# tianrluo/MRphy.py

Hardware: NVIDIA B200
Metric: spin_steps_per_sec_fwd_bwd (higher is better)
Workload: dtype f32

## Files before the change

mrphy.py_b200/csrc/blochsim_fused.cu:

```cuda
#include <cuda_runtime.h>
#include <stdint.h>
#include <stdio.h>
#include <stdlib.h>
#include <string.h>

#include "../../include/mrphy_b200.h"
#include "abi_common.cuh"
#define MRPHY_VOTE_MASK 0xffffffffu
#ifndef MRPHY_TC_MIN_NC
#define MRPHY_TC_MIN_NC 4
#endif
#include "bloch_math.cuh"
#include "ptx_helpers.cuh"
#include "tc_helpers.cuh"
#include "grad_finalize.cuh"

namespace mrphy {

#ifndef MRPHY_TCMAX1
#define MRPHY_TCMAX1 128
#endif
constexpr int TCMAX = 64;
template <typename T, int NC> struct ChunkMax { static constexpr int v = (sizeof(T) == 4 && NC == 1) ? MRPHY_TCMAX1 : TCMAX; };

#ifdef MRPHY_CTA_TRACE
__device__ unsigned long long g_cta_trace[8192][4];
__device__ __forceinline__ unsigned long long gtime() {
  unsigned long long t;
  asm volatile("mov.u64 %0, %globaltimer;" : "=l"(t));
  return t;
}
__device__ __forceinline__ unsigned smid() {
  unsigned s;
  asm volatile("mov.u32 %0, %smid;" : "=r"(s));
  return s;
}
#endif

template <typename T, int PK> struct Pack { typedef T type; };
template <> struct Pack<float, 2> { typedef f2 type; };

template <typename T, int W> struct WaveLayout {
  static constexpr bool STEPMAJOR = W * sizeof(T) > 44;
  static constexpr int WS = STEPMAJOR ? ((W + 3) & ~3) : W;
};
template <typename T, int W>
__device__ __forceinline__ void load_step(const T* wb, int TCP, int j, T (&sv)[W]) {
  if constexpr (WaveLayout<T, W>::STEPMAJOR) {
    constexpr int WS = WaveLayout<T, W>::WS;
    T tmp[WS];
    const float4* src = reinterpret_cast<const float4*>(wb + (size_t)j * WS);
    float4* dst = reinterpret_cast<float4*>(tmp);
#pragma unroll
    for (int e = 0; e < WS * (int)sizeof(T) / 16; ++e) dst[e] = src[e];
#pragma unroll
    for (int w = 0; w < W; ++w) sv[w] = tmp[w];
  } else {
#pragma unroll
    for (int w = 0; w < W; ++w) sv[w] = wb[w * TCP + j];
  }
}

#ifndef MRPHY_RED_BUDGET
#define MRPHY_RED_BUDGET 10240
#endif
#ifndef MRPHY_NC2_MINB
#define MRPHY_NC2_MINB 14
#endif
#ifndef MRPHY_WRED_TR_BYTES
#define MRPHY_WRED_TR_BYTES 64
#endif
#ifndef MRPHY_MC_MINB
#define MRPHY_MC_MINB 1
#endif
#ifndef MRPHY_BWD_MINB
#define MRPHY_BWD_MINB 8
#endif
#ifndef MRPHY_BWD_BLKT
#define MRPHY_BWD_BLKT 128
#endif
constexpr int pick_tr(int W, int elem) {
  int tr = 16;
  const int budget = W >= 19 ? 2 * MRPHY_RED_BUDGET : (W == 11 ? MRPHY_RED_BUDGET + 1024 : (W == 7 ? MRPHY_RED_BUDGET + 4096 : MRPHY_RED_BUDGET));
  while (tr > 1 && W * tr * 32 * elem > budget) tr >>= 1;
  return tr;
}

template <typename T, int NC, int BLKT, int PK = 1> struct BwdSmem {
  static constexpr int W = 2 * NC + 3;
  static constexpr int NW = BLKT / 32;
  static constexpr bool WRED = NC > 1 && PK == 1;
  static constexpr int TR = WRED ? MRPHY_WRED_TR_BYTES / (int)sizeof(T) : pick_tr(W, (int)sizeof(T));
  static constexpr int WP = (W + 3) & ~3;
  static constexpr int E16 = (int)sizeof(T) / 4;
  static constexpr int P16 = TR * E16 + 1;
  static constexpr size_t red_bytes = WRED ? (size_t)NW * 32 * (P16 * 16 + WP * sizeof(T)) : (size_t)NW * W * TR * 32 * sizeof(T);
  static constexpr size_t wbuf = 0;
  static constexpr int WS = WaveLayout<T, W>::WS;
  static constexpr int TCM = ChunkMax<T, NC>::v;
  static constexpr size_t red = (2 * WS * TCM * sizeof(T) + 127) / 128 * 128;
  static constexpr size_t cta = (red + red_bytes + 15) / 16 * 16;
  static constexpr size_t bar = (cta + (size_t)2 * NW * W * TR * sizeof(T) + 15) / 16 * 16;
  static constexpr size_t bytes = bar + 16;
};

template <typename T> struct KArgs {
  int N, nM, nT, K, TCP, nChunks, P;
  int chunk_elems;
  const T* Mi; int64_t Mi_sn, Mi_sm;
  const T* loc; int64_t loc_sn, loc_sm;
  const T* b1; int64_t b1_sn, b1_sm; int nC;
  mrphy_param df, T1, T2, gamma, dt;
  T* Mo;
  T* ckpt;
  const T* wave;
  const T* gMo; int64_t gMo_sn, gMo_sm;
  T* gMi;
  T* partials;
  int* sched;
  int n_sm, c_per_sm;
  int* done;
};
template <typename T> struct SgOut {
  T* gloc; T* gsz; T* gb1;
  bool any() const { return gloc || gsz || gb1; }
};
template <typename T> struct RecOut {
  T* Mt; const T* gMt;
  int every, nR;
};

constexpr int SCHED_SM_SLOTS = 256;
constexpr int SCHED_NCLAIMED = 256;
constexpr int SCHED_CLAIM = 264;
__device__ __forceinline__ unsigned my_smid() {
  unsigned s;
  asm volatile("mov.u32 %0, %%smid;" : "=r"(s));
  return s;
}

__device__ __forceinline__ void load4(const float* p, float (&v)[4]) {
  const float4 q = *reinterpret_cast<const float4*>(p);
  v[0] = q.x; v[1] = q.y; v[2] = q.z; v[3] = q.w;
}
__device__ __forceinline__ void load4(const double* p, double (&v)[4]) {
  const double2 a = *reinterpret_cast<const double2*>(p);
  const double2 b = *reinterpret_cast<const double2*>(p + 2);
  v[0] = a.x; v[1] = a.y; v[2] = b.x; v[3] = b.y;
}

template <int Q> __device__ __forceinline__ float getq(f2 a) { return Q == 0 ? a.v.x : a.v.y; }
template <int Q> __device__ __forceinline__ float getq(float a) { return a; }
template <int Q> __device__ __forceinline__ double getq(double a) { return a; }
__device__ __forceinline__ f2 mkv(float a, float b, f2*) { return f2(a, b); }
__device__ __forceinline__ float mkv(float a, float, float*) { return a; }
__device__ __forceinline__ double mkv(double a, double, double*) { return a; }

template <typename T, int NC, bool RELAX>
__device__ __forceinline__ void load_spin(const KArgs<T>& a, int n, int i, T lx, T ly, T lz, SpinConst<T, NC>& k) {
  T br[NC], bi[NC];
  if (a.b1) {
    const T* bp = a.b1 + (int64_t)n * a.b1_sn + (int64_t)i * a.b1_sm;
#pragma unroll
    for (int c = 0; c < NC; ++c) {
      br[c] = c < a.nC ? bp[c] : (T)0;
      bi[c] = c < a.nC ? bp[a.nC + c] : (T)0;
    }
  }
  const double gam = ld_param(a.gamma, n, i);
  const double dt = ld_param(a.dt, n, 0);
  const double df = a.df.ptr ? ld_param(a.df, n, i) : 0.0;
  const double t1 = RELAX ? ld_param(a.T1, n, i) : 1.0;
  const double t2 = RELAX ? ld_param(a.T2, n, i) : 1.0;
  make_consts<T, NC>(k, gam, dt, RELAX, t1, t2, df, lx, ly, lz, a.b1 ? br : nullptr, a.b1 ? bi : nullptr);
}
template <typename T, typename V, int NC, int PK, bool RELAX>
__device__ __forceinline__ void load_consts_v(const KArgs<T>& a, int n, const int (&idx)[PK], V lx, V ly, V lz,
                                              SpinConst<V, NC>& k) {
  if constexpr (PK == 1) {
    load_spin<T, NC, RELAX>(a, n, idx[0], lx, ly, lz, k);
  } else {
    SpinConst<float, NC> k0, k1;
    load_spin<float, NC, RELAX>(a, n, idx[0], getq<0>(lx), getq<0>(ly), getq<0>(lz), k0);
    load_spin<float, NC, RELAX>(a, n, idx[1], getq<1>(lx), getq<1>(ly), getq<1>(lz), k1);
    k = pack2<NC>(k0, k1);
  }
}
template <typename T, typename V, int PK>
__device__ __forceinline__ void load_vec3(const T* base, int64_t stride, const int (&idx)[PK], V& x, V& y, V& z) {
  const T* p0 = base + (int64_t)idx[0] * stride;
  const T* p1 = base + (int64_t)idx[PK - 1] * stride;
  x = mkv(p0[0], p1[0], (V*)nullptr);
  y = mkv(p0[1], p1[1], (V*)nullptr);
  z = mkv(p0[2], p1[2], (V*)nullptr);
}

template <typename T, typename V, int PK, int BLKT>
__device__ __forceinline__ void load_vec3_tile(const T* base, int64_t stride, int tile, int nM, const int (&idx)[PK],
                                               T* scr, V& x, V& y, V& z) {
  constexpr int TILE = BLKT * PK;
  const T* src = base + (int64_t)tile * TILE * 3;
  const bool coop = stride == 3 && (tile + 1) * TILE <= nM && (reinterpret_cast<uintptr_t>(src) & 15) == 0;
  if (coop) {
    constexpr int NVEC = TILE * 3 * (int)sizeof(T) / 16;
    const float4* s4 = reinterpret_cast<const float4*>(src);
    float4* d4 = reinterpret_cast<float4*>(scr);
    for (int q = threadIdx.x; q < NVEC; q += BLKT) d4[q] = s4[q];
    __syncthreads();
    const int l0 = threadIdx.x, l1 = (PK - 1) * BLKT + threadIdx.x;
    x = mkv(scr[3 * l0], scr[3 * l1], (V*)nullptr);
    y = mkv(scr[3 * l0 + 1], scr[3 * l1 + 1], (V*)nullptr);
    z = mkv(scr[3 * l0 + 2], scr[3 * l1 + 2], (V*)nullptr);
    __syncthreads();
  } else {
    load_vec3<T, V, PK>(base, stride, idx, x, y, z);
  }
}

template <typename T, typename V, int PK>
__device__ __forceinline__ void rec_store(const RecOut<T>& o, int nM, int n, int r, const int (&idx)[PK], const bool (&ok)[PK],
                                          V x, V y, V z) {
  T* p = o.Mt + ((size_t)n * o.nR + r) * 3 * (size_t)nM;
  if (ok[0]) {
    __stcs(p + idx[0], getq<0>(x));
    __stcs(p + (size_t)nM + idx[0], getq<0>(y));
    __stcs(p + 2 * (size_t)nM + idx[0], getq<0>(z));
  }
  if (PK == 2 && ok[PK - 1]) {
    __stcs(p + idx[PK - 1], getq<1>(x));
    __stcs(p + (size_t)nM + idx[PK - 1], getq<1>(y));
    __stcs(p + 2 * (size_t)nM + idx[PK - 1], getq<1>(z));
  }
}
template <typename T, typename V, int NC, int PK>
__device__ __forceinline__ void rec_load(const RecOut<T>& o, int nM, int n, int r, const int (&idx)[PK], const bool (&ok)[PK],
                                         const SpinConst<V, NC>& k, V& x, V& y, V& z) {
  const T* p = o.gMt + ((size_t)n * o.nR + r) * 3 * (size_t)nM;
  T v[PK][3];
#pragma unroll
  for (int q = 0; q < PK; ++q) {
#pragma unroll
    for (int e = 0; e < 3; ++e) v[q][e] = ok[q] ? __ldcs(p + e * (size_t)nM + idx[q]) : (T)0;
  }
  x = mkv(v[0][0], v[PK - 1][0], (V*)nullptr);
  y = mkv(v[0][1], v[PK - 1][1], (V*)nullptr);
  z = mkv(v[0][2], v[PK - 1][2], (V*)nullptr);
  to_frame(k, x, y);
}

template <typename T>
__global__ void pack_waveform_kernel(const T* __restrict__ rf, int64_t rf_sn, int64_t rf_sx, int64_t rf_st, int64_t rf_sc,
                                     const T* __restrict__ gr, int64_t gr_sn, int64_t gr_sx, int64_t gr_st, int nC,
                                     int NC, int sum_coils, int nT, int K, int TCP, int nChunks, int WS, int stepmajor,
                                     int64_t total, T* __restrict__ wave) {
  const int W = 2 * NC + 3;
  for (int64_t e = (int64_t)blockIdx.x * blockDim.x + threadIdx.x; e < total; e += (int64_t)gridDim.x * blockDim.x) {
    const int j = stepmajor ? (int)((e / WS) % TCP) : (int)(e % TCP);
    const int w = stepmajor ? (int)(e % WS) : (int)((e / TCP) % WS);
    const int c = (int)((e / ((int64_t)TCP * WS)) % nChunks);
    const int n = (int)(e / ((int64_t)TCP * WS * nChunks));
    const int t = c * K + j;
    T v = (T)0;
    if (j < K && t < nT && w < W) {
      if (w < 2 * NC) {
        const int x = w / NC, coil = w % NC;
        const T* p = rf + n * rf_sn + x * rf_sx + t * rf_st;
        if (sum_coils) {
          for (int q = 0; q < nC; ++q) v += p[q * rf_sc];
        } else if (coil < nC) {
          v = p[coil * rf_sc];
        }
      } else {
        v = gr[n * gr_sn + (w - 2 * NC) * gr_sx + t * gr_st];
      }
    }
    wave[e] = v;
  }
}

template <typename T, int POL, bool RELAX, int NC, int PK, int BLKT, bool REC = false>
__global__ void __launch_bounds__(BLKT, (PK == 2 ? (NC == 1 ? 14 : MRPHY_NC2_MINB) : 1)) fused_fwd_kernel(const KArgs<T> a, const RecOut<T> rec) {
  typedef typename Pack<T, PK>::type V;
  constexpr int W = 2 * NC + 3;
  constexpr int WS = WaveLayout<T, W>::WS;
  __shared__ __align__(128) T wbuf[2][WS * ChunkMax<T, NC>::v];
  __shared__ __align__(16) T scr[3 * BLKT * PK];
  __shared__ __align__(8) uint64_t full[2];
  const int tid = threadIdx.x, n = blockIdx.y;
  const int TCP = a.TCP, K = a.K, nT = a.nT, nChunks = a.nChunks, nM = a.nM;
  const uint32_t chunk_bytes = (uint32_t)(WS * TCP * sizeof(T));
  const T* wave_n = a.wave + (size_t)n * nChunks * WS * TCP;
  const int tiles = (nM + BLKT * PK - 1) / (BLKT * PK);
  const int my_tiles = ((int)blockIdx.x < tiles) ? (tiles - (int)blockIdx.x + (int)gridDim.x - 1) / (int)gridDim.x : 0;
  const uint32_t total = (uint32_t)my_tiles * (uint32_t)nChunks;
  if (tid == 0) {
    mbar_init(&full[0], 1);
    mbar_init(&full[1], 1);
    fence_barrier_init();
  }
  __syncthreads();
  if (tid == 0 && total > 0) {
    mbar_arrive_expect_tx(&full[0], chunk_bytes);
    bulk_g2s(wbuf[0], wave_n, chunk_bytes, &full[0]);
  }
  uint32_t it = 0;
  for (int tile = blockIdx.x; tile < tiles; tile += gridDim.x) {
    SpinConst<V, NC> k;
    V mx, my, mz;
    int idx[PK];
    bool ok[PK];
#pragma unroll
    for (int q = 0; q < PK; ++q) {
      const int i = (tile * PK + q) * BLKT + tid;
      ok[q] = i < nM;
      idx[q] = ok[q] ? i : nM - 1;
    }
    {
      V lx, ly, lz;
      load_vec3_tile<T, V, PK, BLKT>(a.loc + (int64_t)n * a.loc_sn, a.loc_sm, tile, nM, idx, scr, lx, ly, lz);
      load_consts_v<T, V, NC, PK, RELAX>(a, n, idx, lx, ly, lz, k);
    }
    load_vec3_tile<T, V, PK, BLKT>(a.Mi + (int64_t)n * a.Mi_sn, a.Mi_sm, tile, nM, idx, scr, mx, my, mz);
    to_frame(k, mx, my);
    int rc = rec.every, rr = 0;
    for (int c = 0; c < nChunks; ++c, ++it) {
      if (tid == 0 && it + 1 < total) {
        const int cn = (c + 1 == nChunks) ? 0 : c + 1;
        const uint32_t sn = (it + 1) & 1;
        mbar_arrive_expect_tx(&full[sn], chunk_bytes);
        bulk_g2s(wbuf[sn], wave_n + (size_t)cn * WS * TCP, chunk_bytes, &full[sn]);
      }
      mbar_wait(&full[it & 1], (it >> 1) & 1);
      const T* wb = wbuf[it & 1];
      const int ns = min(K, nT - c * K);
      auto one_step = [&](const T (&s)[W]) {
        V rx[NC], ry[NC], bx, by, bz;
#pragma unroll
        for (int q = 0; q < NC; ++q) { rx[q] = V(s[q]); ry[q] = V(s[NC + q]); }
        field<V, NC>(k, rx, ry, V(s[2 * NC]), V(s[2 * NC + 1]), V(s[2 * NC + 2]), bx, by, bz);
        step_fwd<V, POL, RELAX>(bx, by, bz, k.e1, k.e2, mx, my, mz);
        if constexpr (REC) {
          if (--rc == 0) {
            V x = mx, y = my;
            from_frame(k, x, y);
            rec_store<T, V, PK>(rec, nM, n, rr++, idx, ok, x, y, mz);
            rc = rec.every;
          }
        }
      };
      int j = 0;
      constexpr bool VEC4 = !WaveLayout<T, W>::STEPMAJOR;
      for (; VEC4 && j + 4 <= ns; j += 4) {
        T wv[W][4];
#pragma unroll
        for (int w = 0; w < W; ++w) load4(wb + w * TCP + j, wv[w]);
#pragma unroll
        for (int u = 0; u < 4; ++u) {
          T s[W];
#pragma unroll
          for (int w = 0; w < W; ++w) s[w] = wv[w][u];
          one_step(s);
        }
      }
      for (; j < ns; ++j) {
        T s[W];
        load_step<T, W>(wb, TCP, j, s);
        one_step(s);
      }
      if (c + 1 < nChunks) {
        T* cp = a.ckpt + ((size_t)n * (nChunks - 1) + c) * 3 * (size_t)nM;
        if (ok[0]) {
          __stcs(cp + idx[0], getq<0>(mx));
          __stcs(cp + (size_t)nM + idx[0], getq<0>(my));
          __stcs(cp + 2 * (size_t)nM + idx[0], getq<0>(mz));
        }
        if (PK == 2 && ok[PK - 1]) {
          __stcs(cp + idx[PK - 1], getq<1>(mx));
          __stcs(cp + (size_t)nM + idx[PK - 1], getq<1>(my));
          __stcs(cp + 2 * (size_t)nM + idx[PK - 1], getq<1>(mz));
        }
      }
      __syncthreads();
    }
    from_frame(k, mx, my);
    if (ok[0]) {
      T* op = a.Mo + ((size_t)n * nM + idx[0]) * 3;
      op[0] = getq<0>(mx); op[1] = getq<0>(my); op[2] = getq<0>(mz);
    }
    if (PK == 2 && ok[PK - 1]) {
      T* op = a.Mo + ((size_t)n * nM + idx[PK - 1]) * 3;
      op[0] = getq<1>(mx); op[1] = getq<1>(my); op[2] = getq<1>(mz);
    }
  }
}

template <typename T, int W, int TR, int W0 = 0, int W1 = W>
__device__ __forceinline__ void warp_tile_reduce(const T (*tile)[TR][32], int lane, T (*out)[TR]) {
  if constexpr (sizeof(T) == 4 && TR == 16) {
    const int r = lane >> 1, half = (lane & 1) << 4;
#pragma unroll
    for (int w = W0; w < W1; ++w) {
      const float4* row = reinterpret_cast<const float4*>(&tile[w][r][half]);
      T sum = (T)0;
#pragma unroll
      for (int q = 0; q < 4; ++q) {
        const float4 v = row[(q + r) & 3];
        sum += (v.x + v.y) + (v.z + v.w);
      }
      sum += __shfl_xor_sync(0xffffffffu, sum, 1);
      if (!(lane & 1)) out[w][r] = sum;
    }
  } else {
    const int r = lane & (TR - 1), grp = lane & ~(TR - 1);
#pragma unroll
    for (int w = W0; w < W1; ++w) {
      T sum = (T)0;
#pragma unroll
      for (int q = 0; q < TR; ++q) sum += tile[w][r][grp + ((q + lane) & (TR - 1))];
#pragma unroll
      for (int o = TR; o < 32; o <<= 1) sum += __shfl_xor_sync(0xffffffffu, sum, o);
      if (lane < TR) out[w][r] = sum;
    }
  }
}

template <typename T, int NC, int TR, int W0, int W1>
__device__ __forceinline__ void warp_tile_reduce_weighted(const unsigned char* ft, const T* wt, int lane, T (*out)[TR]) {
  constexpr int W = 2 * NC + 3, WP = (W + 3) & ~3, E16 = (int)sizeof(T) / 4, P16 = TR * E16 + 1, SP = TR;
  constexpr bool WANT_RF = W0 == 0, WANT_GR = W1 == W;
  const int r = lane % TR, grp = lane / TR;
  T acc[W];
#pragma unroll
  for (int w = 0; w < W; ++w) acc[w] = (T)0;
#pragma unroll 2
  for (int q = 0; q < SP; ++q) {
    const int sp = grp * SP + q;
    T f[4];
    {
      const float4* src = reinterpret_cast<const float4*>(ft + ((size_t)sp * P16 + (size_t)r * E16) * 16);
      float4* dst = reinterpret_cast<float4*>(f);
#pragma unroll
      for (int e = 0; e < E16; ++e) dst[e] = src[e];
    }
    T wv[WP];
    {
      const float4* src = reinterpret_cast<const float4*>(wt + (size_t)sp * WP);
      float4* dst = reinterpret_cast<float4*>(wv);
#pragma unroll
      for (int e = 0; e < WP * (int)sizeof(T) / 16; ++e) dst[e] = src[e];
    }
    if constexpr (WANT_RF) {
#pragma unroll
      for (int c = 0; c < NC; ++c) {
        acc[c] = fma_(wv[c], f[0], fma_(wv[NC + c], f[1], acc[c]));
        acc[NC + c] = fma_(wv[c], f[1], fnma_(wv[NC + c], f[0], acc[NC + c]));
      }
    }
    if constexpr (WANT_GR) {
      acc[2 * NC] = fma_(wv[2 * NC], f[2], acc[2 * NC]);
      acc[2 * NC + 1] = fma_(wv[2 * NC + 1], f[2], acc[2 * NC + 1]);
      acc[2 * NC + 2] = fma_(wv[2 * NC + 2], f[2], acc[2 * NC + 2]);
    }
  }
#pragma unroll
  for (int w = W0; w < W1; ++w) {
    T sum = acc[w];
#pragma unroll
    for (int o = TR; o < 32; o <<= 1) sum += __shfl_xor_sync(0xffffffffu, sum, o);
    if (lane < TR) out[w][r] = sum;
  }
}

template <typename T, typename V, int NC, int PK>
__device__ __forceinline__ void sg_fold(const KArgs<T>& a, const SgOut<T>& o, int n, const int (&idx)[PK], const bool (&ok)[PK], bool first,
                                        bool last, const SpinConst<V, NC>& k, const V (&acc)[4 + 2 * NC]) {
  constexpr int NA = 4 + 2 * NC;
#pragma unroll
  for (int q = 0; q < PK; ++q) {
    if (!ok[q]) continue;
    const size_t s = (size_t)n * a.nM + idx[q];
    T v[NA];
#pragma unroll
    for (int w = 0; w < NA; ++w) v[w] = q == 0 ? getq<0>(acc[w]) : getq<1>(acc[w]);
    T* const pl = o.gloc ? o.gloc + s * 3 : nullptr;
    T* const pz = o.gsz ? o.gsz + s : nullptr;
    T* const pb = o.gb1 ? o.gb1 + s * 2 * a.nC : nullptr;
    if (!first) {
      if (pl) { v[0] += pl[0]; v[1] += pl[1]; v[2] += pl[2]; }
      if (pz) v[3] += pz[0];
      if (pb) {
#pragma unroll
        for (int c = 0; c < NC; ++c)
          if (c < a.nC) { v[4 + c] += pb[c]; v[4 + NC + c] += pb[a.nC + c]; }
      }
    }
    if (last) {
      const T ng = (T)(-6.283185307179586476925286766559 * ld_param(a.gamma, n, idx[q]) * ld_param(a.dt, n, 0));
#pragma unroll
      for (int w = 0; w < NA; ++w) v[w] *= ng;
      if (NC == 1) {
        const T fc = q == 0 ? getq<0>(k.fc) : getq<1>(k.fc), fs = q == 0 ? getq<0>(k.fs) : getq<1>(k.fs);
        const T re = v[4], im = v[5];
        v[4] = fnma_(fs, im, fc * re);
        v[5] = fma_(fs, re, fc * im);
      }
    }
    if (pl) { pl[0] = v[0]; pl[1] = v[1]; pl[2] = v[2]; }
    if (pz) pz[0] = v[3];
    if (pb) {
#pragma unroll
      for (int c = 0; c < NC; ++c)
        if (c < a.nC) { pb[c] = v[4 + c]; pb[a.nC + c] = v[4 + NC + c]; }
    }
  }
}

template <typename T, int POL, bool RELAX, int NC, int PK, int BLKT, int ROWS = 3, bool SG = false, bool REC = false>
__global__ void __launch_bounds__(BLKT, (PK == 2 ? MRPHY_BWD_MINB * 64 / BLKT : (sizeof(T) == 8 && NC == 1 ? 4 : (sizeof(T) == 4 && NC > 1 ? MRPHY_MC_MINB : 1)))) fused_bwd_kernel(const KArgs<T> a, const int need_gmi, const SgOut<T> sgo, const RecOut<T> rec) {
  typedef typename Pack<T, PK>::type V;
  using L = BwdSmem<T, NC, BLKT, PK>;
  constexpr int W = L::W, TR = L::TR, NW = L::NW;
  constexpr bool WANT_RF = (ROWS & 1) != 0, WANT_GR = (ROWS & 2) != 0;
  constexpr int W0 = WANT_RF ? 0 : 2 * NC, W1 = WANT_GR ? W : 2 * NC;
  extern __shared__ __align__(128) unsigned char smem_raw[];
  constexpr int WS = L::WS;
  T(*wbuf)[WS * L::TCM] = reinterpret_cast<T(*)[WS * L::TCM]>(smem_raw + L::wbuf);
  T(*red)[W][TR][32] = reinterpret_cast<T(*)[W][TR][32]>(smem_raw + L::red);
  constexpr bool WRED = L::WRED;
  unsigned char* const ft = smem_raw + L::red + (size_t)(threadIdx.x >> 5) * 32 * L::P16 * 16;
  T* const wt = reinterpret_cast<T*>(smem_raw + L::red + (size_t)NW * 32 * L::P16 * 16) + (size_t)(threadIdx.x >> 5) * 32 * L::WP;
  T(*cta)[W][TR] = reinterpret_cast<T(*)[W][TR]>(smem_raw + L::cta);
  uint64_t* full = reinterpret_cast<uint64_t*>(smem_raw + L::bar);
  __shared__ __align__(16) T scr[3 * BLKT * PK];
  const int tid = threadIdx.x, lane = tid & 31, warp = tid >> 5, n = blockIdx.y;
  const int TCP = a.TCP, K = a.K, nT = a.nT, nChunks = a.nChunks, nM = a.nM;
  const uint32_t chunk_bytes = (uint32_t)(WS * TCP * sizeof(T));
  const T* wave_n = a.wave + (size_t)n * nChunks * WS * TCP;
  const int tiles = (nM + BLKT * PK - 1) / (BLKT * PK);
#define NCTA ((int)gridDim.x)
  __shared__ int s_vid, s_sweep;
  if (tid == 0) {
    mbar_init(&full[0], 1);
    mbar_init(&full[1], 1);
    fence_barrier_init();
  }
  if (a.done && blockIdx.x == 0 && tid == 0) a.done[n] = 0;
  int vid = blockIdx.x;
  if (a.sched && tid == 0) {
    int* const sched = a.sched;
    s_sweep = 0;
    const int s = (int)my_smid();
    int v0 = -1;
    if (s < a.n_sm && s < SCHED_SM_SLOTS) {
      const int rank = atomicAdd(&sched[s], 1);
      const int cand = rank * a.n_sm + s;
      if (rank < a.c_per_sm && cand < NCTA && atomicCAS(&sched[SCHED_CLAIM + cand], 0, 1) == 0) {
        v0 = cand;
        atomicAdd(&sched[SCHED_NCLAIMED], 1);
      }
    }
    s_vid = v0;
  }
  __syncthreads();
  if (a.sched) vid = s_vid;
#ifdef MRPHY_CTA_TRACE
  if (tid == 0 && blockIdx.x < 8192 && n == 0) { g_cta_trace[blockIdx.x][0] = smid(); g_cta_trace[blockIdx.x][1] = gtime(); g_cta_trace[blockIdx.x][3] = (unsigned long long)(long long)vid; }
#endif
  uint32_t it = 0, red_par = 0;
  for (;;) {
   if (vid >= 0) {
    const int my_tiles = (vid < tiles) ? (tiles - vid + NCTA - 1) / NCTA : 0;
    const uint32_t total = it + (uint32_t)my_tiles * (uint32_t)nChunks;
    T* part = a.partials + ((size_t)n * a.P + vid) * W * (size_t)nT;
    if (my_tiles == 0) {
      if constexpr (ROWS != 0)
        for (int e = tid; e < W * nT; e += BLKT) part[e] = (T)0;
    } else if (tid == 0) {
      mbar_arrive_expect_tx(&full[it & 1], chunk_bytes);
      bulk_g2s(wbuf[it & 1], wave_n + (size_t)(nChunks - 1) * WS * TCP, chunk_bytes, &full[it & 1]);
    }
  bool first = true;
  for (int tile = vid; tile < tiles; tile += NCTA, first = false) {
    SpinConst<V, NC> k;
    V mx, my, mz, hx, hy, hz;
    int idx[PK];
    bool ok[PK];
#pragma unroll
    for (int q = 0; q < PK; ++q) {
      const int i = (tile * PK + q) * BLKT + tid;
      ok[q] = i < nM;
      idx[q] = ok[q] ? i : nM - 1;
    }
    {
      V lx, ly, lz;
      load_vec3_tile<T, V, PK, BLKT>(a.loc + (int64_t)n * a.loc_sn, a.loc_sm, tile, nM, idx, scr, lx, ly, lz);
      load_consts_v<T, V, NC, PK, RELAX>(a, n, idx, lx, ly, lz, k);
    }
    load_vec3_tile<T, V, PK, BLKT>(a.Mo + (size_t)n * nM * 3, 3, tile, nM, idx, scr, mx, my, mz);
    load_vec3_tile<T, V, PK, BLKT>(a.gMo + (int64_t)n * a.gMo_sn, a.gMo_sm, tile, nM, idx, scr, hx, hy, hz);
    to_frame(k, mx, my);
    to_frame(k, hx, hy);
    if constexpr (WRED && ROWS != 0) {
      T* wrow = wt + (size_t)lane * L::WP;
#pragma unroll
      for (int q = 0; q < NC; ++q) { wrow[q] = lane0(k.cbr[q]); wrow[NC + q] = lane0(k.cbi[q]); }
      wrow[2 * NC] = lane0(k.glx); wrow[2 * NC + 1] = lane0(k.gly); wrow[2 * NC + 2] = lane0(k.glz);
#pragma unroll
      for (int q = W; q < L::WP; ++q) wrow[q] = (T)0;
      __syncwarp();
    }
    {
      const T z0 = ok[0] ? (T)1 : (T)0, z1 = ok[PK - 1] ? (T)1 : (T)0;
      const V zm = mkv(z0, z1, (V*)nullptr);
      hx = hx * zm; hy = hy * zm; hz = hz * zm;
    }
    int rc = 0, rr = 0;
    V gx, gy, gz;
    if constexpr (REC) {
      rc = nT - rec.nR * rec.every;
      rr = rec.nR - 1;
      rec_load<T, V, NC, PK>(rec, nM, n, rr, idx, ok, k, gx, gy, gz);
    }
    for (int c = nChunks - 1; c >= 0; --c, ++it) {
      if (tid == 0 && it + 1 < total) {
        const int cn = (c == 0) ? nChunks - 1 : c - 1;
        const uint32_t sn = (it + 1) & 1;
        mbar_arrive_expect_tx(&full[sn], chunk_bytes);
        bulk_g2s(wbuf[sn], wave_n + (size_t)cn * WS * TCP, chunk_bytes, &full[sn]);
      }
      V kx = mx, ky = my, kz = mz;
      if (c > 0) {
        const T* cp = a.ckpt + ((size_t)n * (nChunks - 1) + (c - 1)) * 3 * (size_t)nM;
        kx = mkv(__ldcs(cp + idx[0]), __ldcs(cp + idx[PK - 1]), (V*)nullptr);
        ky = mkv(__ldcs(cp + (size_t)nM + idx[0]), __ldcs(cp + (size_t)nM + idx[PK - 1]), (V*)nullptr);
        kz = mkv(__ldcs(cp + 2 * (size_t)nM + idx[0]), __ldcs(cp + 2 * (size_t)nM + idx[PK - 1]), (V*)nullptr);
      }
      mbar_wait(&full[it & 1], (it >> 1) & 1);
      const T* wb = wbuf[it & 1];
      const int ns = min(K, nT - c * K);
      V sacc[SG ? 4 + 2 * NC : 1];
      if constexpr (SG) {
#pragma unroll
        for (int w = 0; w < 4 + 2 * NC; ++w) sacc[w] = V(0.0f);
      }
      auto one_step = [&](const T (&s)[W], int row) {
        if constexpr (REC) {
          if (rc == 0) {
            hx = hx + gx; hy = hy + gy; hz = hz + gz;
            if (--rr >= 0) rec_load<T, V, NC, PK>(rec, nM, n, rr, idx, ok, k, gx, gy, gz);
            rc = rec.every;
          }
          --rc;
        }
        V rx[NC], ry[NC], bx, by, bz, Fx, Fy, Fz;
#pragma unroll
        for (int q = 0; q < NC; ++q) { rx[q] = V(s[q]); ry[q] = V(s[NC + q]); }
        field<V, NC>(k, rx, ry, V(s[2 * NC]), V(s[2 * NC + 1]), V(s[2 * NC + 2]), bx, by, bz);
        step_bwd<V, POL, RELAX, NC>(k, bx, by, bz, mx, my, mz, hx, hy, hz, Fx, Fy, Fz);
        if constexpr (SG) {
          sacc[0] = fma_(V(s[2 * NC]), Fz, sacc[0]);
          sacc[1] = fma_(V(s[2 * NC + 1]), Fz, sacc[1]);
          sacc[2] = fma_(V(s[2 * NC + 2]), Fz, sacc[2]);
          sacc[3] = sacc[3] + Fz;
#pragma unroll
          for (int q = 0; q < NC; ++q) {
            sacc[4 + q] = fma_(rx[q], Fx, fma_(ry[q], Fy, sacc[4 + q]));
            sacc[4 + NC + q] = fma_(rx[q], Fy, fnma_(ry[q], Fx, sacc[4 + NC + q]));
          }
        }
        if constexpr (ROWS == 0) return;
        if constexpr (WRED) {
          T fv[4] = {lane0(Fx), lane0(Fy), lane0(Fz), (T)0};
          float4* dst = reinterpret_cast<float4*>(ft + ((size_t)lane * L::P16 + (size_t)row * L::E16) * 16);
          const float4* src = reinterpret_cast<const float4*>(fv);
#pragma unroll
          for (int e = 0; e < L::E16; ++e) dst[e] = src[e];
          return;
        }
        if constexpr (WANT_RF) {
#pragma unroll
          for (int q = 0; q < NC; ++q) {
            V gx_, gy_;
            rf_chain<V, NC>(k, q, Fx, Fy, gx_, gy_);
            red[warp][q][row][lane] = hsum(gx_);
            red[warp][NC + q][row][lane] = hsum(gy_);
          }
        }
        if constexpr (WANT_GR) {
          red[warp][2 * NC][row][lane] = hsum(k.glx * Fz);
          red[warp][2 * NC + 1][row][lane] = hsum(k.gly * Fz);
          red[warp][2 * NC + 2][row][lane] = hsum(k.glz * Fz);
        }
      };
      for (int j1 = ns; j1 > 0;) {
        const int j0 = ((j1 - 1) / TR) * TR;
        constexpr bool VEC4 = !WaveLayout<T, W>::STEPMAJOR && TR % 4 == 0;
        if (VEC4 && j1 - j0 == TR) {
#pragma unroll 1
          for (int jj = TR - 4; jj >= 0; jj -= 4) {
            T wv[W][4];
#pragma unroll
            for (int w = 0; w < W; ++w) load4(wb + w * TCP + j0 + jj, wv[w]);
#pragma unroll
            for (int u = 3; u >= 0; --u) {
              T s[W];
#pragma unroll
              for (int w = 0; w < W; ++w) s[w] = wv[w][u];
              one_step(s, jj + u);
            }
          }
        } else {
          for (int j = j1 - 1; j >= j0; --j) {
            T s[W];
            load_step<T, W>(wb, TCP, j, s);
            one_step(s, j - j0);
          }
        }
        if constexpr (ROWS != 0) {
        __syncwarp();
        T(*ctab)[W][TR] = cta + (size_t)(red_par & 1) * NW;
        if constexpr (WRED) warp_tile_reduce_weighted<T, NC, TR, W0, W1>(ft, wt, lane, ctab[warp]);
        else warp_tile_reduce<T, W, TR, W0, W1>(red[warp], lane, ctab[warp]);
        __syncthreads();
        for (int e = tid; e < (W1 - W0) * TR; e += BLKT) {
          const int w = W0 + e / TR, r = e % TR;
          if (j0 + r < j1) {
            T sum = ctab[0][w][r];
#pragma unroll
            for (int q = 1; q < NW; ++q) sum += ctab[q][w][r];
            T* dst = part + (size_t)w * nT + (c * K + j0 + r);
            if (first) *dst = sum; else atomicAdd(dst, sum);
          }
        }
        ++red_par;
        }
        j1 = j0;
      }
      if constexpr (SG) sg_fold<T, V, NC, PK>(a, sgo, n, idx, ok, c == nChunks - 1, c == 0, k, sacc);
      if constexpr (ROWS == 0) __syncthreads();
      if (c > 0) {
        mx = kx; my = ky; mz = kz;
      }
    }
    if (need_gmi) {
      from_frame(k, hx, hy);
      if (ok[0]) {
        T* op = a.gMi + ((size_t)n * nM + idx[0]) * 3;
        op[0] = getq<0>(hx); op[1] = getq<0>(hy); op[2] = getq<0>(hz);
      }
      if (PK == 2 && ok[PK - 1]) {
        T* op = a.gMi + ((size_t)n * nM + idx[PK - 1]) * 3;
        op[0] = getq<1>(hx); op[1] = getq<1>(hy); op[2] = getq<1>(hz);
      }
    }
  }
   }
   if (!a.sched) break;
   __syncthreads();
   if (tid == 0) {
     int* const sched = a.sched;
     int f = -1, sweep = s_sweep;
     if (*(volatile int*)&sched[SCHED_NCLAIMED] < NCTA) {
       for (; sweep < NCTA; ++sweep) {
         if (*(volatile int*)&sched[SCHED_CLAIM + sweep] == 0 && atomicCAS(&sched[SCHED_CLAIM + sweep], 0, 1) == 0) {
           f = sweep++;
           atomicAdd(&sched[SCHED_NCLAIMED], 1);
           break;
         }
       }
     }
     s_sweep = sweep;
     s_vid = f;
   }
   __syncthreads();
   vid = s_vid;
   if (vid < 0) break;
  }
#undef NCTA
#ifdef MRPHY_CTA_TRACE
  if (tid == 0 && blockIdx.x < 8192 && n == 0) g_cta_trace[blockIdx.x][2] = gtime();
#endif
}


constexpr int TC_TCMAX = 32;
template <int NC> struct TcLayout {
  static constexpr int KC = NC / 2;
  static constexpr int KSTEPS = NC / 4;
  static constexpr int PER_STEP = 16 * KC + 3;
  static constexpr int CHUNK_MAX = TC_TCMAX * PER_STEP;
  static constexpr int A_FLOATS = 2 * KC * 128 * 4;
  static constexpr int TILE_COLS = 2 * TC_TCMAX;
};
template <int NC, int PK> struct TcCfg {
  static constexpr int NBUF = PK == 1 ? 2 : 1;
  static constexpr int NST = (PK == 1 && NC <= 8) ? 3 : 2;
  static constexpr int BUF_COLS = PK * TcLayout<NC>::TILE_COLS;
  static constexpr int TMEM_COLS = NBUF * BUF_COLS;
  static constexpr size_t wbuf = 0;
  static constexpr size_t sa = ((size_t)NST * TcLayout<NC>::CHUNK_MAX * 4 + 127) / 128 * 128;
  static constexpr size_t scr = sa + (size_t)PK * TcLayout<NC>::A_FLOATS * 4;
  static constexpr size_t bars = scr + (size_t)3 * 128 * PK * 4;
  static constexpr size_t bytes = bars + 64;
};

template <int NC>
__global__ void pack_waveform_tc_kernel(const float* __restrict__ rf, int64_t rf_sn, int64_t rf_sx, int64_t rf_st, int64_t rf_sc,
                                        const float* __restrict__ gr, int64_t gr_sn, int64_t gr_sx, int64_t gr_st, int nC,
                                        int nT, int K, int TCP, int nChunks, int64_t total, float* __restrict__ wave) {
  using L = TcLayout<NC>;
  const int rows = 2 * TCP;
  for (int64_t e = (int64_t)blockIdx.x * blockDim.x + threadIdx.x; e < total; e += (int64_t)gridDim.x * blockDim.x) {
    const int q = (int)(e % NC);
    const int j = (int)((e / NC) % TCP);
    const int c = (int)((e / ((int64_t)NC * TCP)) % nChunks);
    const int n = (int)(e / ((int64_t)NC * TCP * nChunks));
    const int t = c * K + j;
    const bool live = j < K && t < nT;
    float rx = 0.f, ry = 0.f;
    if (live && q < nC) {
      const float* p = rf + n * rf_sn + t * rf_st + q * rf_sc;
      rx = p[0];
      ry = p[rf_sx];
    }
    float* chunk = wave + ((size_t)n * nChunks + c) * (size_t)(TCP * L::PER_STEP);
    const float xh = tc::tf32_rn(rx), xm = tc::tf32_rn(rx - xh), yh = tc::tf32_rn(ry), ym = tc::tf32_rn(ry - yh);
    const int kc = q >> 1, pos = (q & 1) * 2;
    float* b_hi = chunk + ((size_t)(0 * L::KC + kc) * rows) * 4 + pos;
    float* b_mid = chunk + ((size_t)(1 * L::KC + kc) * rows) * 4 + pos;
    *reinterpret_cast<float2*>(b_hi + (size_t)(2 * j) * 4) = make_float2(xh, -yh);
    *reinterpret_cast<float2*>(b_hi + (size_t)(2 * j + 1) * 4) = make_float2(yh, xh);
    *reinterpret_cast<float2*>(b_mid + (size_t)(2 * j) * 4) = make_float2(xm, -ym);
    *reinterpret_cast<float2*>(b_mid + (size_t)(2 * j + 1) * 4) = make_float2(ym, xm);
    if (q < 3) chunk[(size_t)2 * L::KC * rows * 4 + (size_t)q * TCP + j] = live ? gr[n * gr_sn + q * gr_sx + t * gr_st] : 0.f;
  }
}

template <int NC, bool RELAX>
__device__ __forceinline__ void tc_load_spin(const KArgs<float>& a, int n, int i, float lx, float ly, float lz,
                                             SpinConst<float, 1>& k, float* sa, int tid) {
  using L = TcLayout<NC>;
  const double gam = ld_param(a.gamma, n, i);
  const double dt = ld_param(a.dt, n, 0);
  const double df = a.df.ptr ? ld_param(a.df, n, i) : 0.0;
  const double t1 = RELAX ? ld_param(a.T1, n, i) : 1.0;
  const double t2 = RELAX ? ld_param(a.T2, n, i) : 1.0;
  make_consts<float, 1>(k, gam, dt, RELAX, t1, t2, df, lx, ly, lz, nullptr, nullptr);
  const double g = 6.283185307179586476925286766559 * gam * dt;
  const float* bp = a.b1 + (int64_t)n * a.b1_sn + (int64_t)i * a.b1_sm;
#pragma unroll 2
  for (int kc = 0; kc < L::KC; ++kc) {
    float v[4], h[4], m[4];
#pragma unroll
    for (int e = 0; e < 2; ++e) {
      const int c = 2 * kc + e;
      v[2 * e] = c < a.nC ? (float)(g * (double)bp[c]) : 0.f;
      v[2 * e + 1] = c < a.nC ? (float)(g * (double)bp[a.nC + c]) : 0.f;
    }
#pragma unroll
    for (int e = 0; e < 4; ++e) { h[e] = tc::tf32_rn(v[e]); m[e] = tc::tf32_rn(v[e] - h[e]); }
    *reinterpret_cast<float4*>(sa + ((size_t)(0 * L::KC + kc) * 128 + tid) * 4) = make_float4(h[0], h[1], h[2], h[3]);
    *reinterpret_cast<float4*>(sa + ((size_t)(1 * L::KC + kc) * 128 + tid) * 4) = make_float4(m[0], m[1], m[2], m[3]);
  }
  fence_proxy_async_smem();
}
template <int NC, int PK>
__device__ __forceinline__ void tc_issue(const float* sa, const float* wb, int rows, uint32_t tmem, uint64_t* bar) {
  using L = TcLayout<NC>;
  const uint32_t idesc = tc::idesc_tf32(128, rows);
  const int pa[3] = {1, 0, 0}, pb[3] = {0, 1, 0};
  tc::fence_after_sync();
#pragma unroll
  for (int t = 0; t < PK; ++t) {
    bool acc = false;
#pragma unroll
    for (int q = 0; q < 3; ++q) {
#pragma unroll
      for (int ks = 0; ks < L::KSTEPS; ++ks) {
        tc::mma_tf32(tmem + t * L::TILE_COLS, tc::kmajor_desc(sa + (size_t)t * L::A_FLOATS + ((size_t)(pa[q] * L::KC + 2 * ks) * 128) * 4, 128),
                     tc::kmajor_desc(wb + ((size_t)(pb[q] * L::KC + 2 * ks) * rows) * 4, rows), idesc, acc);
        acc = true;
      }
    }
  }
  tc::commit(bar);
}

#define TC_CHUNK_BEGIN(CHUNK_OF, FIRST_OF_TILE, HAS_NEXT_IN_TILE)                                                          \
  if (tid == 0) {                                                                                                          \
    if (it + (NST - 1) < total) {                                                                                          \
      const uint32_t sq = (it + (NST - 1)) % NST;                                                                          \
      mbar_arrive_expect_tx(&full[sq], chunk_bytes);                                                                       \
      bulk_g2s(wbuf[sq], wave_n + (size_t)(CHUNK_OF(it + (NST - 1))) * a.chunk_elems, chunk_bytes, &full[sq]);              \
    }                                                                                                                      \
    if ((FIRST_OF_TILE) || NBUF == 1) {                                                                                    \
      mbar_wait(&full[it % NST], (it / NST) & 1);                                                                          \
      tc_issue<NC, PK>(sa, wbuf[it % NST], rows, tmem + (it % NBUF) * C::BUF_COLS, &mma_bar[it % NBUF]);                    \
    }                                                                                                                      \
    if (NBUF == 2 && NST == 3 && (HAS_NEXT_IN_TILE)) {                                                                     \
      mbar_wait(&full[(it + 1) % NST], ((it + 1) / NST) & 1);                                                              \
      tc_issue<NC, PK>(sa, wbuf[(it + 1) % NST], rows, tmem + ((it + 1) % NBUF) * C::BUF_COLS, &mma_bar[(it + 1) % NBUF]);  \
    }                                                                                                                      \
  }                                                                                                                        \
  mbar_wait(&full[it % NST], (it / NST) & 1);                                                                              \
  mbar_wait(&mma_bar[it % NBUF], (it / NBUF) & 1);                                                                         \
  tc::fence_after_sync();
#define TC_PRODUCT_AHEAD(HAS_NEXT_IN_TILE)                                                                                 \
  if (NBUF == 2 && NST == 2 && tid == 0 && (HAS_NEXT_IN_TILE)) {                                                           \
    mbar_wait(&full[(it + 1) % NST], ((it + 1) / NST) & 1);                                                                \
    tc_issue<NC, PK>(sa, wbuf[(it + 1) % NST], rows, tmem + ((it + 1) % NBUF) * C::BUF_COLS, &mma_bar[(it + 1) % NBUF]);    \
  }

template <int POL, bool RELAX, int NC, int PK, bool REC = false>
__global__ void __launch_bounds__(128, (NC <= 8 ? 4 : (PK == 1 ? 3 : 2))) fused_fwd_tc_kernel(const KArgs<float> a, const RecOut<float> rec) {
  using L = TcLayout<NC>;
  using C = TcCfg<NC, PK>;
  typedef float T;
  typedef typename Pack<float, PK>::type V;
  constexpr int BLKT = 128, NST = C::NST, NBUF = C::NBUF;
  extern __shared__ __align__(128) unsigned char smem_raw[];
  float(*wbuf)[L::CHUNK_MAX] = reinterpret_cast<float(*)[L::CHUNK_MAX]>(smem_raw + C::wbuf);
  float* const sa = reinterpret_cast<float*>(smem_raw + C::sa);
  float* const scr = reinterpret_cast<float*>(smem_raw + C::scr);
  uint64_t* const full = reinterpret_cast<uint64_t*>(smem_raw + C::bars);
  uint64_t* const mma_bar = full + NST;
  uint32_t* const tmem_slot = reinterpret_cast<uint32_t*>(full + NST + 2);
  const int tid = threadIdx.x, warp = tid >> 5, n = blockIdx.y;
  const int TCP = a.TCP, K = a.K, nT = a.nT, nChunks = a.nChunks, nM = a.nM, rows = 2 * TCP;
  const uint32_t chunk_bytes = (uint32_t)(a.chunk_elems * sizeof(float));
  const float* wave_n = a.wave + (size_t)n * nChunks * a.chunk_elems;
  const int tiles = (nM + BLKT * PK - 1) / (BLKT * PK);
  const int my_tiles = ((int)blockIdx.x < tiles) ? (tiles - (int)blockIdx.x + (int)gridDim.x - 1) / (int)gridDim.x : 0;
  const uint32_t total = (uint32_t)my_tiles * (uint32_t)nChunks;
  if (tid == 0) {
#pragma unroll
    for (int q = 0; q < NST; ++q) mbar_init(&full[q], 1);
    mbar_init(&mma_bar[0], 1);
    mbar_init(&mma_bar[1], 1);
    fence_barrier_init();
  }
  if (warp == 0) tc::tmem_alloc<C::TMEM_COLS>(tmem_slot);
  tc::fence_before_sync();
  __syncthreads();
  tc::fence_after_sync();
  const uint32_t tmem = *tmem_slot, tlane = tmem + ((uint32_t)(warp * 32) << 16);
#define FWD_CHUNK_OF(i) ((i) % (uint32_t)nChunks)
  if (tid == 0) {
    for (uint32_t q = 0; q + 1 < (uint32_t)NST && q < total; ++q) {
      mbar_arrive_expect_tx(&full[q], chunk_bytes);
      bulk_g2s(wbuf[q], wave_n + (size_t)FWD_CHUNK_OF(q) * a.chunk_elems, chunk_bytes, &full[q]);
    }
  }
  uint32_t it = 0;
  for (int tile = blockIdx.x; tile < tiles; tile += gridDim.x) {
    SpinConst<V, 1> k;
    V mx, my, mz;
    int idx[PK];
    bool ok[PK];
#pragma unroll
    for (int q = 0; q < PK; ++q) {
      const int i = (tile * PK + q) * BLKT + tid;
      ok[q] = i < nM;
      idx[q] = ok[q] ? i : nM - 1;
    }
    {
      V lx, ly, lz;
      load_vec3_tile<T, V, PK, BLKT>(a.loc + (int64_t)n * a.loc_sn, a.loc_sm, tile, nM, idx, scr, lx, ly, lz);
      if constexpr (PK == 1) {
        tc_load_spin<NC, RELAX>(a, n, idx[0], lx, ly, lz, k, sa, tid);
      } else {
        SpinConst<float, 1> k0, k1;
        tc_load_spin<NC, RELAX>(a, n, idx[0], getq<0>(lx), getq<0>(ly), getq<0>(lz), k0, sa, tid);
        tc_load_spin<NC, RELAX>(a, n, idx[1], getq<1>(lx), getq<1>(ly), getq<1>(lz), k1, sa + L::A_FLOATS, tid);
        k = pack2<1>(k0, k1);
      }
    }
    load_vec3_tile<T, V, PK, BLKT>(a.Mi + (int64_t)n * a.Mi_sn, a.Mi_sm, tile, nM, idx, scr, mx, my, mz);
    tc::fence_before_sync();
    __syncthreads();
    const V glx = k.glx, gly = k.gly, glz = k.glz, gbz0 = k.gbz0, e1 = k.e1, e2 = k.e2;
    int rc = rec.every, rr = 0;
    for (int c = 0; c < nChunks; ++c, ++it) {
      TC_CHUNK_BEGIN(FWD_CHUNK_OF, c == 0, c + 1 < nChunks)
      const float* gw = wbuf[it % NST] + (size_t)2 * L::KC * rows * 4;
      const int ns = min(K, nT - c * K);
      const uint32_t tcol = tlane + (it % NBUF) * C::BUF_COLS;
      auto steps8 = [&](const float (&b)[PK][16], int j0) {
        float g[3][8];
#pragma unroll
        for (int w = 0; w < 3; ++w) {
          load4(gw + w * TCP + j0, *reinterpret_cast<float(*)[4]>(&g[w][0]));
          load4(gw + w * TCP + j0 + 4, *reinterpret_cast<float(*)[4]>(&g[w][4]));
        }
#pragma unroll
        for (int u = 0; u < 8; ++u) {
          if (j0 + u < ns) {
            const V bz = fma_(glx, V(g[0][u]), fma_(gly, V(g[1][u]), fma_(glz, V(g[2][u]), gbz0)));
            const V bx = mkv(b[0][2 * u], b[PK - 1][2 * u], (V*)nullptr), by = mkv(b[0][2 * u + 1], b[PK - 1][2 * u + 1], (V*)nullptr);
            step_fwd<V, POL, RELAX>(bx, by, bz, e1, e2, mx, my, mz);
            if constexpr (REC) {
              if (--rc == 0) {
                rec_store<T, V, PK>(rec, nM, n, rr++, idx, ok, mx, my, mz);
                rc = rec.every;
              }
            }
          }
        }
      };
      auto issue = [&](float (&b)[PK][16], int g) {
#pragma unroll
        for (int q = 0; q < PK; ++q) tc::tmem_ld16_issue(tcol + q * L::TILE_COLS + 16 * g, b[q]);
      };
      auto wait = [&](float (&b)[PK][16]) {
        tc::tmem_ld_wait(b[0]);
        if constexpr (PK == 2) tc::tmem_ld_wait(b[1]);
      };
      float b0[PK][16], b1[PK][16];
      issue(b0, 0);
#pragma unroll 1
      for (int g = 0; g < TC_TCMAX / 8; g += 2) {
        if (8 * g < ns) {
          wait(b0);
          if (8 * (g + 1) < ns) issue(b1, g + 1);
          steps8(b0, 8 * g);
          if (ns <= 8) { TC_PRODUCT_AHEAD(c + 1 < nChunks) }
        }
        if (8 * (g + 1) < ns) {
          wait(b1);
          if (g + 2 < TC_TCMAX / 8 && 8 * (g + 2) < ns) issue(b0, g + 2);
          steps8(b1, 8 * (g + 1));
          if (g == 0) { TC_PRODUCT_AHEAD(c + 1 < nChunks) }
        }
      }
      if (c + 1 < nChunks) {
        T* cp = a.ckpt + ((size_t)n * (nChunks - 1) + c) * 3 * (size_t)nM;
        if (ok[0]) {
          __stcs(cp + idx[0], getq<0>(mx));
          __stcs(cp + (size_t)nM + idx[0], getq<0>(my));
          __stcs(cp + 2 * (size_t)nM + idx[0], getq<0>(mz));
        }
        if (PK == 2 && ok[PK - 1]) {
          __stcs(cp + idx[PK - 1], getq<1>(mx));
          __stcs(cp + (size_t)nM + idx[PK - 1], getq<1>(my));
          __stcs(cp + 2 * (size_t)nM + idx[PK - 1], getq<1>(mz));
        }
      }
// ... 538 lines not shown
```

Baseline: 186.5 billion.

## Add packed-pair staged reduction path for single-coil PK=2 backward kernel

For the NC==1, PK==2 backward kernel, per-step RF gradient partials and raw Fz pairs are now staged in a padded per-lane shared-memory tile. A new warp_tile_reduce_pk2 reduces them, applying the gradient weights (glx/gly/glz, stored once per lane) during the reduction. Before this, each step did three hsum products for the gradient rows and wrote them to the per-row red array. The aim is to cut per-step shared stores and multiplies, at the cost of a different smem layout and extra reduction-time loads. A compile-time probe mode and a SASS comparison script are also added but are off by default.

```diff
diff --git a/mrphy.py_b200/csrc/blochsim_fused.cu b/mrphy.py_b200/csrc/blochsim_fused.cu
--- a/mrphy.py_b200/csrc/blochsim_fused.cu
+++ b/mrphy.py_b200/csrc/blochsim_fused.cu
@@ -79,6 +79,9 @@
 #ifndef MRPHY_BWD_BLKT
 #define MRPHY_BWD_BLKT 128
 #endif
+#ifndef MRPHY_BWD_RED_PROBE
+#define MRPHY_BWD_RED_PROBE 0
+#endif
 constexpr int pick_tr(int W, int elem) {
   int tr = 16;
   const int budget = W >= 19 ? 2 * MRPHY_RED_BUDGET : (W == 11 ? MRPHY_RED_BUDGET + 1024 : (W == 7 ? MRPHY_RED_BUDGET + 4096 : MRPHY_RED_BUDGET));
@@ -90,11 +93,12 @@
   static constexpr int W = 2 * NC + 3;
   static constexpr int NW = BLKT / 32;
   static constexpr bool WRED = NC > 1 && PK == 1;
+  static constexpr bool PRED = NC == 1 && PK == 2;
   static constexpr int TR = WRED ? MRPHY_WRED_TR_BYTES / (int)sizeof(T) : pick_tr(W, (int)sizeof(T));
-  static constexpr int WP = (W + 3) & ~3;
+  static constexpr int WP = PRED ? 8 : (W + 3) & ~3;
   static constexpr int E16 = (int)sizeof(T) / 4;
   static constexpr int P16 = TR * E16 + 1;
-  static constexpr size_t red_bytes = WRED ? (size_t)NW * 32 * (P16 * 16 + WP * sizeof(T)) : (size_t)NW * W * TR * 32 * sizeof(T);
+  static constexpr size_t red_bytes = (WRED || PRED) ? (size_t)NW * 32 * (P16 * 16 + WP * sizeof(T)) : (size_t)NW * W * TR * 32 * sizeof(T);
   static constexpr size_t wbuf = 0;
   static constexpr int WS = WaveLayout<T, W>::WS;
   static constexpr int TCM = ChunkMax<T, NC>::v;
@@ -471,6 +475,39 @@
   }
 }
 
+template <int TR, bool WANT_RF, bool WANT_GR>
+__device__ __forceinline__ void warp_tile_reduce_pk2(const unsigned char* ft, const float* wt, int lane, float (*out)[TR]) {
+  constexpr int P16 = TR + 1, SP = TR;
+  const int r = lane % TR, grp = lane / TR;
+  float ax = 0.f, ay = 0.f;
+  f2 gx(0.f), gy(0.f), gz(0.f);
+#pragma unroll 4
+  for (int q = 0; q < SP; ++q) {
+    const int sp = grp * SP + q;
+    const float4 v = *reinterpret_cast<const float4*>(ft + ((size_t)sp * P16 + r) * 16);
+    if constexpr (WANT_RF) {
+      ax += v.x;
+      ay += v.y;
+    }
+    if constexpr (WANT_GR) {
+      const float4 w0 = *reinterpret_cast<const float4*>(wt + (size_t)sp * 8);
+      const float4 w1 = *reinterpret_cast<const float4*>(wt + (size_t)sp * 8 + 4);
+      const f2 fz(v.z, v.w);
+      gx = fma_(f2(w0.x, w0.y), fz, gx);
+      gy = fma_(f2(w0.z, w0.w), fz, gy);
+      gz = fma_(f2(w1.x, w1.y), fz, gz);
+    }
+  }
+  float s[5] = {ax, ay, hsum(gx), hsum(gy), hsum(gz)};
+#pragma unroll
+  for (int w = WANT_RF ? 0 : 2; w < (WANT_GR ? 5 : 2); ++w) {
+    float sum = s[w];
+#pragma unroll
+    for (int o = TR; o < 32; o <<= 1) sum += __shfl_xor_sync(0xffffffffu, sum, o);
+    if (lane < TR) out[w][r] = sum;
+  }
+}
+
 template <typename T, typename V, int NC, int PK>
 __device__ __forceinline__ void sg_fold(const KArgs<T>& a, const SgOut<T>& o, int n, const int (&idx)[PK], const bool (&ok)[PK], bool first,
                                         bool last, const SpinConst<V, NC>& k, const V (&acc)[4 + 2 * NC]) {
@@ -522,6 +559,8 @@
   constexpr int W = L::W, TR = L::TR, NW = L::NW;
   constexpr bool WANT_RF = (ROWS & 1) != 0, WANT_GR = (ROWS & 2) != 0;
   constexpr int W0 = WANT_RF ? 0 : 2 * NC, W1 = WANT_GR ? W : 2 * NC;
+  constexpr bool PRED = L::PRED, PROBE = PRED && MRPHY_BWD_RED_PROBE != 0;
+  constexpr bool REDUCE = ROWS != 0 && !PROBE;
   extern __shared__ __align__(128) unsigned char smem_raw[];
   constexpr int WS = L::WS;
   T(*wbuf)[WS * L::TCM] = reinterpret_cast<T(*)[WS * L::TCM]>(smem_raw + L::wbuf);
@@ -609,6 +648,16 @@
       for (int q = W; q < L::WP; ++q) wrow[q] = (T)0;
       __syncwarp();
     }
+    if constexpr (PRED && WANT_GR && REDUCE) {
+      float4* wrow = reinterpret_cast<float4*>(wt + (size_t)lane * L::WP);
+      wrow[0] = make_float4(getq<0>(k.glx), getq<1>(k.glx), getq<0>(k.gly), getq<1>(k.gly));
+      wrow[1] = make_float4(getq<0>(k.glz), getq<1>(k.glz), 0.f, 0.f);
+      __syncwarp();
+    }
+#if MRPHY_BWD_RED_PROBE
+    float psink = 0.f;
+    V vsink = V(0.0f);
+#endif
     {
       const T z0 = ok[0] ? (T)1 : (T)0, z1 = ok[PK - 1] ? (T)1 : (T)0;
       const V zm = mkv(z0, z1, (V*)nullptr);
@@ -669,12 +718,32 @@
           }
         }
         if constexpr (ROWS == 0) return;
+#if MRPHY_BWD_RED_PROBE
+        if constexpr (PROBE && MRPHY_BWD_RED_PROBE == 1) {
+          psink += hsum(k.cbr[0] * Fx) + hsum(k.cbr[0] * Fy) + hsum(k.glx * Fz) + hsum(k.gly * Fz) + hsum(k.glz * Fz);
+          return;
+        }
+        if constexpr (PROBE) {
+          vsink = fma_(Fx, Fy, vsink + Fz);
+          return;
+        }
+#endif
         if constexpr (WRED) {
           T fv[4] = {lane0(Fx), lane0(Fy), lane0(Fz), (T)0};
           float4* dst = reinterpret_cast<float4*>(ft + ((size_t)lane * L::P16 + (size_t)row * L::E16) * 16);
           const float4* src = reinterpret_cast<const float4*>(fv);
 #pragma unroll
           for (int e = 0; e < L::E16; ++e) dst[e] = src[e];
+          return;
+        }
+        if constexpr (PRED) {
+          float* dst = reinterpret_cast<float*>(ft + ((size_t)lane * L::P16 + (size_t)row) * 16);
+          if constexpr (ROWS == 3)
+            *reinterpret_cast<float4*>(dst) = make_float4(hsum(k.cbr[0] * Fx), hsum(k.cbr[0] * Fy), getq<0>(Fz), getq<1>(Fz));
+          else if constexpr (ROWS == 1)
+            *reinterpret_cast<float2*>(dst) = make_float2(hsum(k.cbr[0] * Fx), hsum(k.cbr[0] * Fy));
+          else
+            *reinterpret_cast<float2*>(dst + 2) = make_float2(getq<0>(Fz), getq<1>(Fz));
           return;
         }
         if constexpr (WANT_RF) {
@@ -716,10 +785,11 @@
             one_step(s, j - j0);
           }
         }
-        if constexpr (ROWS != 0) {
+        if constexpr (REDUCE) {
         __syncwarp();
         T(*ctab)[W][TR] = cta + (size_t)(red_par & 1) * NW;
         if constexpr (WRED) warp_tile_reduce_weighted<T, NC, TR, W0, W1>(ft, wt, lane, ctab[warp]);
+        else if constexpr (PRED) warp_tile_reduce_pk2<TR, WANT_RF, WANT_GR>(ft, wt, lane, ctab[warp]);
         else warp_tile_reduce<T, W, TR, W0, W1>(red[warp], lane, ctab[warp]);
         __syncthreads();
         for (int e = tid; e < (W1 - W0) * TR; e += BLKT) {
@@ -737,11 +807,16 @@
         j1 = j0;
       }
       if constexpr (SG) sg_fold<T, V, NC, PK>(a, sgo, n, idx, ok, c == nChunks - 1, c == 0, k, sacc);
-      if constexpr (ROWS == 0) __syncthreads();
+      if constexpr (!REDUCE) __syncthreads();
       if (c > 0) {
         mx = kx; my = ky; mz = kz;
       }
     }
+#if MRPHY_BWD_RED_PROBE
+    if constexpr (PROBE) {
+      if (need_gmi == -1) a.gMi[idx[0]] = psink + hsum(vsink);
+    }
+#endif
     if (need_gmi) {
       from_frame(k, hx, hy);
       if (ok[0]) {
diff --git a/profiles/sass_compare.py b/profiles/sass_compare.py
--- /dev/null
+++ b/profiles/sass_compare.py
@@ -0,0 +1,54 @@
+#!/usr/bin/env python
+import hashlib
+import re
+import subprocess
+import sys
+
+
+def sass(lib):
+    out = subprocess.run(['cuobjdump', '-sass', lib], capture_output=True, text=True, check=True).stdout
+    body, cur = {}, None
+    for line in out.splitlines():
+        m = re.match(r'\s*Function : (\S+)', line)
+        if m:
+            cur = m.group(1)
+            body[cur] = []
+        elif cur is not None:
+            m = re.match(r'\s*/\*[0-9a-f]{4,}\*/\s*(.*)', line)
+            if m:
+                body[cur].append(m.group(1))
+            elif re.match(r'\s*/\* 0x[0-9a-f]+ \*/', line):
+                body[cur].append(line.strip())
+    return {k: hashlib.sha256('\n'.join(v).encode()).hexdigest() for k, v in body.items()}
+
+
+def ptxas(path):
+    res, cur = {}, None
+    for line in open(path):
+        m = re.search(r"Compiling entry function '(\S+)'", line)
+        if m:
+            cur = m.group(1)
+        elif cur and ('spill stores' in line or 'Used' in line):
+            res.setdefault(cur, []).append(line.strip().split(': ')[-1])
+            if 'Used' in line:
+                cur = None
+    return {k: ' | '.join(v) for k, v in res.items()}
+
+
+def main():
+    a, b = sass(sys.argv[1]), sass(sys.argv[2])
+    same = sorted(k for k in a if a[k] == b.get(k))
+    diff = sorted(k for k in a if k in b and a[k] != b[k])
+    print(f'kernels: old {len(a)}, new {len(b)}; byte-identical SASS {len(same)}; different {len(diff)}; '
+          f'only in old {len(set(a) - set(b))}; only in new {len(set(b) - set(a))}')
+    pa, pb = (ptxas(sys.argv[3]), ptxas(sys.argv[4])) if len(sys.argv) > 4 else ({}, {})
+    for k in diff:
+        print(f'different {k}')
+        if k in pa or k in pb:
+            print(f'    old: {pa.get(k, "?")}\n    new: {pb.get(k, "?")}')
+    for k in sorted(set(a) ^ set(b)):
+        print(f'only in one {k}')
+
+
+if __name__ == '__main__':
+    main()
```

Result: no change. 188.2 billion, median of 6 (+0.9%).
